# marcelm/cutadapt

Hardware: NVIDIA H100
Metric: reads/sec (150bp SE, 1 adapter, e=0.1) (higher is better)
Workload: dtype u8

## Files before the change

### __graft_entry__.py

```python
import os
import subprocess
import sys

ROOT = os.path.dirname(os.path.abspath(__file__))
CSRC = os.path.join(ROOT, "cutadapt_b200", "csrc")
LIB = os.path.join(ROOT, "cutadapt_b200", "libcutadapt_b200.so")
SOURCES = ["cg_kernels.cu", "cg_fastq.cu", "cg_gzip.cu", "cg_gunzip.cu", "cg_bam.cu", "cg_api.cu", "cg_setbuild.cpp", "cg_host_algos.cpp", "cg_hostpack.cpp", "cg_jit.cpp"]
JIT_HEADERS = ["cg_types.h", "cg_core.cuh", "cg_args.h", "cg_device.cuh", "cg_pscan.cuh"]
HEADERS = ["cg_types.h", "cg_core.cuh", "cg_args.h", "cg_device.cuh", "cg_pscan.cuh", "cg_fastq_core.cuh", "cg_gzip_core.cuh", "cg_gunzip_core.cuh", "cg_bam_core.cuh", "cg_names_core.cuh", "cg_kernels.cuh", "cg_setbuild.h", "cg_hostpack.h", "../../include/cutadapt_b200.h"]


def _newer(target, deps):
    if not os.path.exists(target):
        return True
    t = os.path.getmtime(target)
    return any(os.path.getmtime(d) > t for d in deps if os.path.exists(d))


def write_jit_embed():
    out = os.path.join(CSRC, "cg_jit_embed.h")
    parts = ["// generated by __graft_entry__.write_jit_embed() from " + ", ".join(JIT_HEADERS) + " -- do not edit\n"]
    for i, h in enumerate(JIT_HEADERS):
        text = open(os.path.join(CSRC, h)).read()
        parts.append(f"static const char cg_jit_text_{i}[] =\n")
# ... 33 lines not shown
                print(" ".join(cmd))
            procs.append((cmd, subprocess.Popen(cmd)))
    for cmd, pr in procs:
        if pr.wait() != 0:
            raise subprocess.CalledProcessError(pr.returncode, cmd)
    if force or procs or _newer(LIB, objs):
        subprocess.check_call([nvcc, "-gencode", "arch=compute_90a,code=sm_90a", "-shared", "-o", LIB] + objs
                              + ["-lpthread", "-ldl"])
    return LIB


def build_hostsim(force=False):
    out = os.path.join(ROOT, "tests", "hostsim", "libhostsim.so")
    write_jit_embed()
    srcs = [os.path.join(ROOT, "tests", "hostsim", "hostsim.cpp"), os.path.join(ROOT, "tests", "hostsim", "hostsim_fasta.cpp"),
            os.path.join(ROOT, "tests", "hostsim", "hostsim_route.cpp"),
            os.path.join(ROOT, "tests", "hostsim", "hostsim_pairs.cpp"), os.path.join(ROOT, "tests", "hostsim", "hostsim_gzip.cpp"),
            os.path.join(ROOT, "tests", "hostsim", "hostsim_gunzip.cpp"),
            os.path.join(ROOT, "tests", "hostsim", "hostsim_gunzip_blocks.cpp"),
            os.path.join(ROOT, "tests", "hostsim", "hostsim_quality.cpp"),
            os.path.join(ROOT, "tests", "hostsim", "hostsim_revcomp.cpp"),
            os.path.join(ROOT, "tests", "hostsim", "hostsim_bam.cpp"),
            os.path.join(ROOT, "tests", "hostsim", "hostsim_names.cpp"),
            os.path.join(CSRC, "cg_setbuild.cpp"),
            os.path.join(CSRC, "cg_jit.cpp")]
    deps = srcs + [os.path.join(CSRC, h) for h in ("cg_types.h", "cg_core.cuh", "cg_fastq_core.cuh", "cg_gzip_core.cuh", "cg_gunzip_core.cuh", "cg_bam_core.cuh", "cg_names_core.cuh", "cg_setbuild.h",
                                                   "cg_jit.h", "cg_jit_embed.h")]
    if force or _newer(out, deps):
        subprocess.check_call(["g++", "-O2", "-std=c++17", "-DCG_RUN_BAND=1", "-shared", "-fPIC", "-o", out] + srcs + ["-ldl"])
    return out


def build(force=False):
    build_library(force)
    sys.path.insert(0, ROOT)
    from oracle import oracle as _oracle

    _oracle.build(force)
    build_hostsim(force)
    if os.path.isdir(os.path.join(os.environ.get("CUTADAPT_REFERENCE", ""), "src", "cutadapt")):
        from oracle import build_ref

        build_ref.build()
    import cutadapt_b200
    from cutadapt_b200 import _lib

# ... 42 lines not shown
```

### cutadapt_b200/_lib.py

```python
import ctypes as C
import os
import threading
from typing import Iterable, List, Optional, Sequence, Tuple

import numpy as np

_HERE = os.path.dirname(os.path.abspath(__file__))
LIB_PATH = os.path.join(_HERE, "libcutadapt_b200.so")

CG_OK = 0
CG_EINVAL = -1
CG_ENONASCII = -2
CG_ECUDA = -3
CG_ENOMEM = -4
CG_EUNSUPPORTED = -5
CG_ENOQUAL = -6

CG_KIND_ALIGNER = 0
CG_KIND_PREFIX_COMPARER = 1
CG_KIND_SUFFIX_COMPARER = 2
CG_REMOVE_BEFORE = 0
CG_REMOVE_AFTER = 1
CG_REMOVE_AUTO = 2
CG_GROUP_SINGLE = 0
# ... 201 lines not shown
    lib.cg_fastq_submit_gzip_paired.argtypes = [vp, i32, i32, vp, i64, vp, i64, i32, i32, C.POINTER(i32), C.POINTER(i32),
                                                C.POINTER(cg_gzin_result), C.POINTER(cg_gzin_result)]
    lib.cg_fastq_submit_gzip_interleaved.argtypes = [vp, i32, vp, i64, i32, i32, C.POINTER(i32), C.POINTER(i32),
                                                     C.POINTER(cg_gzin_result)]
    lib.cg_fastq_collect_paired_interleaved.argtypes = [vp, i32, i32, vp, vp, C.POINTER(cg_fastq_params),
                                                        C.POINTER(cg_fastq_params), i32, i32, i32, i32, vp, i64, vp, i64,
                                                        C.POINTER(cg_fastq_result), C.POINTER(cg_fastq_result), vp, vp]
    lib.cg_fastq_stats_create.argtypes = [vp, i32, C.POINTER(i32)]
    lib.cg_fastq_stats_read.argtypes = [vp, i32, C.POINTER(i32), C.POINTER(i32), vp, i64, C.POINTER(i64), C.c_int]
    lib.cg_fastq_stats_destroy.argtypes = [vp, i32]
    lib.cg_names_create.argtypes = [vp, C.POINTER(cg_names_desc), C.POINTER(i32)]
    lib.cg_names_set_mate.argtypes = [vp, i32, i32, C.c_char_p, vp, i32, vp, i32, i32]
    lib.cg_names_destroy.argtypes = [vp, i32]
    lib.cg_adapterset_create.argtypes = [
        vp, C.POINTER(cg_adapter_desc), i32, C.POINTER(cg_group_desc), i32, C.POINTER(vp),
    ]
    lib.cg_adapterset_create_indexed.argtypes = [
        vp, C.POINTER(cg_adapter_desc), i32, C.POINTER(cg_group_desc), i32,
        C.POINTER(cg_index_desc), i32, C.POINTER(vp),
    ]
    lib.cg_adapterset_destroy.argtypes = [vp]
    lib.cg_ctx_stage_times.argtypes = [vp, C.POINTER(C.c_double), C.c_int]
    lib.cg_adapterset_jit_status.argtypes = [vp]
    lib.cg_adapterset_jit_source.argtypes = [vp, C.c_int32, C.c_int32, C.c_int32, C.c_char_p, C.c_int64]
    lib.cg_adapterset_jit_source.restype = C.c_int64
    lib.cg_adapterset_slots.argtypes = [vp]
    lib.cg_adapterset_effective_length.argtypes = [vp, i32, C.POINTER(i32)]
    lib.cg_process_batch.argtypes = [vp, vp, vp, vp, vp, i64, C.POINTER(cg_params), vp, vp]
    lib.cg_process_batch_device.argtypes = [
        vp, vp, vp, vp, vp, i64, i32, C.POINTER(cg_params), vp, vp,
    ]
    lib.cg_process_batch_device_stats.argtypes = [
        vp, vp, vp, vp, vp, i64, i32, C.POINTER(cg_params), vp, vp, i32, i32, vp,
    ]
    lib.cg_kmers_present_batch.argtypes = [vp, C.POINTER(cg_kmer_entry), vp, i32, vp, vp, i64, vp]
    lib.cg_quality_trim_batch.argtypes = [vp, vp, vp, i64, i32, i32, i32, vp]
    lib.cg_nextseq_trim_batch.argtypes = [vp, vp, vp, vp, i64, i32, i32, vp]
    lib.cg_poly_a_trim_batch.argtypes = [vp, vp, vp, i64, i32, vp]
    lib.cg_expected_errors_batch.argtypes = [vp, vp, vp, i64, i32, vp]
    lib.cg_stats_size.argtypes = [i32, i32, i32]
    lib.cg_stats_size.restype = i64
    lib.cg_stats_accumulate_device.argtypes = [
        vp, vp, vp, vp, i64, C.POINTER(cg_params), vp, vp, i32, i32, vp,
    ]
    lib.cg_locate_debug.argtypes = [vp, C.POINTER(cg_adapter_desc), vp, i32, vp, vp, vp]
    lib.cg_process_batch_stats.argtypes = [vp, vp, vp, vp, vp, i64, C.POINTER(cg_params), vp, vp, i32, i32, vp]
    lib.cg_edit_environment.argtypes = [vp, i32, i32, i32, vp, vp, vp, vp, i64]
# ... 315 lines not shown

class AdapterSet:

    def __init__(self, spec: AdapterSetSpec, ctx: Optional[Context] = None):
        self.spec = spec
        self.ctx = ctx or default_context()
        arr, n, garr, ng = spec.to_ctypes()
        handle = C.c_void_p()
        iarr, ni = spec.index_ctypes()
        if ni:
            check(lib().cg_adapterset_create_indexed(self.ctx.handle, arr, n, garr, ng, iarr, ni, C.byref(handle)))
        else:
            check(lib().cg_adapterset_create(self.ctx.handle, arr, n, garr, ng, C.byref(handle)))
        self._h = handle
        self.slots = int(lib().cg_adapterset_slots(handle))

    @property
    def handle(self):
        return self._h

    def jit_status(self) -> int:
        return int(lib().cg_adapterset_jit_status(self._h))

    def jit_source(self, plane_words: int = 5, has_qual: bool = False, statistics: bool = False) -> str:
        n = int(lib().cg_adapterset_jit_source(self._h, plane_words, int(has_qual), int(statistics), None, 0))
        if n == 0:
            return ""
        buf = C.create_string_buffer(n + 1)
        lib().cg_adapterset_jit_source(self._h, plane_words, int(has_qual), int(statistics), buf, n + 1)
        return buf.value.decode()

    def effective_length(self, adapter: int = 0) -> int:
        out = C.c_int32()
        check(lib().cg_adapterset_effective_length(self._h, adapter, C.byref(out)))
        return out.value

    def process(
        self,
        seq: np.ndarray,
        offsets: np.ndarray,
        qual: Optional[np.ndarray] = None,
        params: Optional[cg_params] = None,
        want_qtrim: bool = False,
    ):
        params = params or make_params()
        n = int(offsets.size - 1)
        seq = np.ascontiguousarray(seq, dtype=np.uint8)
        offsets = np.ascontiguousarray(offsets, dtype=np.int64)
        if (params.quality_trim or params.nextseq_trim) and qual is None:
            from .qualtrim import HasNoQualities

            raise HasNoQualities("Cannot do quality trimming when no qualities are available")
# ... 28 lines not shown
```

### cutadapt_b200/csrc/cg_api.cu

```cuda
#include <cuda_runtime.h>
#include <stdio.h>
#include <stdlib.h>
#include <ctype.h>
#include <string.h>

#include <algorithm>
#include <chrono>
#include <map>
#include <memory>
#include <string>
#include <type_traits>
#include <vector>

#include "../../include/cutadapt_b200.h"
#include "cg_hostpack.h"
#include <array>

#include "cg_gzip_core.cuh"
#include "cg_kernels.cuh"
#include "cg_jit.h"
#include "cg_setbuild.h"

static_assert(sizeof(cg_match) == 32 && sizeof(cg_match_rec) == 32, "cg_match must be 32 bytes");
static_assert(sizeof(CgAdapter) == 80 && sizeof(CgEntry) == 32 && sizeof(CgGroup) == 32 &&
// ... 228 lines not shown
    std::map<int32_t, GzinStream> gzin;
    std::map<int32_t, NamesProg> names;
    int32_t names_next = 1;
    int32_t gzin_next = 1;
};

struct cg_adapterset {
    cg_ctx *ctx = nullptr;
    CgBuiltSet host;
    uint8_t *d_blob = nullptr;
    uint64_t *d_masks = nullptr;
    CgEntry *d_entries = nullptr;
    uint8_t *d_index = nullptr;
    struct Pass {
        cg_adapterset *sub = nullptr;
        int group = 0, role = 0;
        int front_pass = -1;
        int map_off = 0;
    };
    std::vector<Pass> passes;
    std::vector<int32_t> pass_map;
    int32_t *d_pass_map = nullptr;
    CgSelectTables select_tables;
    mutable CgJitKernel *jit[2][2][2] = {};
    mutable int jit_state[2][2][2] = {};
    mutable long long plane_reads = 0;
    mutable std::string jit_error;
};

extern "C" int cg_ctx_create(int device, void *stream, cg_ctx **out)
{
    if (!out) return fail(CG_EINVAL, "cg_ctx_create: out is NULL");
    int count = 0;
    cudaError_t e = cudaGetDeviceCount(&count);
    if (e != cudaSuccess || count == 0)
        return fail(CG_ECUDA, std::string("no usable CUDA device (") + cudaGetErrorString(e) +
                                  "); cutadapt_b200 has no CPU fallback");
    if (device < 0 || device >= count) return fail(CG_EINVAL, "cg_ctx_create: device ordinal out of range");
    CU(cudaSetDevice(device));
    std::unique_ptr<cg_ctx, decltype(&cg_ctx_destroy)> c(new cg_ctx(), cg_ctx_destroy);
    c->device = device;
    cudaDeviceProp prop;
    CU(cudaGetDeviceProperties(&prop, device));
    c->sm_count = prop.multiProcessorCount;
    c->smem_optin = prop.sharedMemPerBlockOptin;
    if (stream) { c->stream = (cudaStream_t)stream; c->own_stream = false; }
    else { CU(cudaStreamCreateWithFlags(&c->stream, cudaStreamNonBlocking)); c->own_stream = true; }
    for (int i = 0; i < CG_N_LANES; ++i) CU(cudaStreamCreateWithFlags(&c->lanes[i].stream, cudaStreamNonBlocking));
// ... 155 lines not shown
            if (e == cudaSuccess)
                e = cudaMemcpy(s->d_pass_map, s->pass_map.data(), s->pass_map.size() * sizeof(int32_t), cudaMemcpyHostToDevice);
            if (e != cudaSuccess) { cudaGetLastError(); ok = false; }
        }
        if (!ok) destroy_passes(s);
    }
    *out = s;
    return CG_OK;
}

extern "C" int cg_adapterset_create(cg_ctx *c, const cg_adapter_desc *adapters, int32_t n_adapters,
                                    const cg_group_desc *groups, int32_t n_groups, cg_adapterset **out)
{
    return cg_adapterset_create_indexed(c, adapters, n_adapters, groups, n_groups, nullptr, 0, out);
}

extern "C" int cg_adapterset_destroy(cg_adapterset *s)
{
    if (!s) return CG_OK;
    if (s->ctx) cudaSetDevice(s->ctx->device);
    if (s->d_blob) cudaFree(s->d_blob);
    if (s->d_masks) cudaFree(s->d_masks);
    if (s->d_index) cudaFree(s->d_index);
    for (int w = 0; w < 2; ++w)
        for (int q = 0; q < 2; ++q)
            for (int v = 0; v < 2; ++v) cg_jit_destroy(s->jit[w][q][v]);
    destroy_passes(s);
    delete s;
    return CG_OK;
}

extern "C" int cg_adapterset_jit_status(const cg_adapterset *s)
{
    if (!s) return 0;
    const cg_adapterset *t = (!s->passes.empty() && s->passes[0].sub) ? s->passes[0].sub : s;
    int st = 0;
    for (int w = 0; w < 2; ++w)
        for (int q = 0; q < 2; ++q)
            for (int v = 0; v < 2; ++v) {
                if (t->jit_state[w][q][v] == 1) st = 1;
                else if (t->jit_state[w][q][v] == -1 && st == 0) st = -1;
            }
    if (st == -1) g_err = "first-stage specialisation failed: " + t->jit_error;
    return st;
}

extern "C" int64_t cg_adapterset_jit_source(const cg_adapterset *s, int32_t plane_words, int32_t has_qual, int32_t stats,
                                            char *buf, int64_t cap)
{
    if (!s) return 0;
    const std::string src = cg_jit_pscan_source(s->host, plane_words, has_qual != 0, stats != 0);
    if (buf && cap > 0) {
        const size_t n = std::min<size_t>(src.size(), (size_t)cap - 1);
        memcpy(buf, src.data(), n);
        buf[n] = 0;
    }
    return (int64_t)src.size();
}

extern "C" int cg_adapterset_slots(const cg_adapterset *s) { return s ? s->host.slots : 0; }

extern "C" int cg_adapterset_effective_length(const cg_adapterset *s, int32_t adapter, int32_t *out)
{
    if (!s || !out || adapter < 0 || adapter >= s->host.n_adapters) return fail(CG_EINVAL, "bad adapter index");
    *out = s->host.effective_length[adapter];
    return CG_OK;
}

struct TrimSwitches {
    static bool is(const char *name, const char *value) { const char *e = getenv(name); return e && strcmp(e, value) == 0; }
    static long long at_least_1024(const char *e) { const long long v = e ? atoll(e) : 0; return v >= 1024 ? v : 0; }
    bool force_general = is("CUTADAPT_B200_KERNEL", "general");
    bool force_block = is("CUTADAPT_B200_KERNEL", "block");
    bool force_warp = is("CUTADAPT_B200_KERNEL", "warp");
// ... 75 lines not shown
    d.mini_cap = (int)mini;
    d.carry_slot = (int)(d.plane_w ? std::max<long long>(cslot, 16LL * (2 * d.plane_w + 1) + 16) : cslot);
    size_t scan_smem = d.plane_w ? cg_pscan_smem_bytes(blob_bytes, d.mini_cap, want_q)
                                 : cg_scan_smem_bytes(blob_bytes, d.mini_cap, want_q);
    d.list_smem = cg_dp_smem_bytes(blob_bytes, d.carry_slot);
    if (scan_smem > c->smem_optin || d.list_smem > c->smem_optin) return CG_OK;
    int scan_occ = 0;
    if (d.plane_w) CU(cg_pscan_occupancy(want_q, d.plane_w, false, scan_smem, &scan_occ));
    else CU(cg_scan_occupancy(want_q, scan_smem, &scan_occ));
    CU(cg_list_occupancy(true, h.max_m, false, d.list_smem, &d.plan_occ));
    CU(cg_list_occupancy(false, h.max_m, false, d.list_smem, &d.run_occ));
    if (scan_occ < 1 || d.plan_occ < 1 || d.run_occ < 1) return CG_OK;
    if (d.plane_w && stats && !has_view && h.n_adapters == 1 && times == 1 && h.slots == 1 && !want_q && !sw.two_lists &&
        stats->max_len <= 4096 && cg_stats_entries_smem_bytes(stats->max_len, stats->kmax) <= 48 * 1024) {
        const size_t fsmem = cg_pscan_smem_bytes(blob_bytes, d.mini_cap, want_q, stats->max_len);
        int focc = 0;
        if (fsmem <= c->smem_optin) CU(cg_pscan_occupancy(want_q, d.plane_w, true, fsmem, &focc));
        int pocc = 0, rocc = 0;
        CU(cg_list_occupancy(true, h.max_m, true, d.list_smem, &pocc));
        CU(cg_list_occupancy(false, h.max_m, true, d.list_smem, &rocc));
        d.fuse_stats = focc >= 1 && focc >= scan_occ && pocc >= d.plan_occ && rocc >= d.run_occ;
        if (d.fuse_stats) { scan_smem = fsmem; scan_occ = focc; }
    }
    if (d.plane_w) {
        const int wi = d.plane_w <= 5 ? 0 : 1, qi = want_q ? 1 : 0, vi = d.fuse_stats ? 1 : 0;
        s->plane_reads += n_reads;
        if (!sw.jit_never && s->jit_state[wi][qi][vi] == 0 && (sw.jit_always || s->plane_reads >= (4LL << 20))) {
            std::string err;
            s->jit[wi][qi][vi] = cg_jit_build_pscan(h, d.plane_w, want_q, d.fuse_stats, err);
            s->jit_state[wi][qi][vi] = s->jit[wi][qi][vi] ? 1 : -1;
            if (!s->jit[wi][qi][vi]) s->jit_error = err;
        }
        if (!sw.jit_never && s->jit_state[wi][qi][vi] == 1) {
            d.jit_occ = cg_jit_occupancy(s->jit[wi][qi][vi], CG_NT, scan_smem);
            if (d.jit_occ >= 1) d.jit = s->jit[wi][qi][vi];
        }
    }
    d.kind = TrimKind::Split;
    d.smem = scan_smem; d.occ = scan_occ;
    d.sub = sw.sub_reads ? sw.sub_reads : (d.plane_w && sw.task_bytes) ? (16LL << 20) : (32LL << 20);
    d.sub = std::min<long long>(d.sub, 1LL << 31);
    d.plane_rec = d.plane_w ? (sw.task_bytes ? 4 + 2 * d.plane_w + 1 : 4) : 2;
    return CG_OK;
}

static int trim_grid(const cg_ctx *c, int blocks_per_sm, long long need)
{
    return (int)std::max<long long>(1, std::min<long long>((long long)blocks_per_sm * c->sm_count, need));
}

static int launch_index(cg_ctx *c, const CgKernelArgs &a, const TrimSchedule &d, cudaStream_t st)
{
    int rc = c->tasks.ensure((size_t)((std::min<long long>(a.n_reads, d.sub) + 3) / 4));
    if (rc != CG_OK) return rc;
    for (long long r0 = 0; r0 < a.n_reads; r0 += d.sub) {
        const long long n_sub = std::min<long long>(d.sub, a.n_reads - r0);
        CgKernelArgs b = a;
        b.offsets = a.offsets + r0; b.n_reads = n_sub; b.out = a.out + (size_t)r0 * a.slots;
// ... 3379 lines not shown
```

### cutadapt_b200/csrc/cg_core.cuh

```cuda
#pragma once
#include "cg_types.h"

#define CGK_KIND_ALIGNER 0
#define CGK_KIND_PREFIX 1
#define CGK_KIND_SUFFIX 2
#define CGK_REMOVE_BEFORE 0
#define CGK_REMOVE_AFTER 1
#define CGK_REMOVE_AUTO 2
#define CGK_GROUP_SINGLE 0
#define CGK_GROUP_LINKED 1
#define CGK_GROUP_INDEXED 2

CG_HD int cg_ctz(uint32_t x)
{
#if defined(__CUDA_ARCH__)
    return __ffs((int)x) - 1;
#else
    return __builtin_ctz(x);
#endif
}
CG_HD uint32_t cg_funnel_r(uint32_t lo, uint32_t hi, uint32_t shift_bits)
{
#if defined(__CUDA_ARCH__)
    return __funnelshift_r(lo, hi, shift_bits);
// ... 728 lines not shown
        const int e_min = 32 * W - window + len - 1;
#pragma unroll
        for (int b = 0; b < W; ++b) {
            const int fv = e_min - 32 * b;
            x[b] &= fv <= 0 ? 0xFFFFFFFFu : (fv >= 32 ? 0u : (0xFFFFFFFFu << fv));
        }
#pragma unroll
        for (int b = (W >= 3 ? W - 3 : 0); b < W; ++b) any |= x[b];
    } else {
#pragma unroll
        for (int b = 0; b < W; ++b) any |= x[b];
    }
    if ((flags & (int)CG_PLANE_GUARD) && any) st.guard = true;
    if ((flags & (int)CG_PLANE_PASS) && any) st.pass = true;
    if (flags & (int)CG_PLANE_LOC) {
        if (any) st.anyhit = true;
        if (plane_shl<W>(x, (uint32_t)shift)) st.end_hit = true;
#pragma unroll
        for (int b = 0; b < W; ++b) { st.M[b] |= x[b]; st.E[b] &= x[b]; }
    }
}

struct RuntimePlaneProg {
    CG_HD static bool same_adapter(const uint8_t *w, const uint8_t *ref, int m)
    {
        bool same = true;
        for (int i = 0; i < m; ++i) same = same && ((w[i] & 0xDFu) == ref[i]);
        return same;
    }
    CG_HD static int adapter_length(int m) { return m; }
    CG_HD static unsigned long long overlap_ok(unsigned long long from_blob) { return from_blob; }
    CG_HD static int remove_kind(int from_blob) { return from_blob; }
    template <int W>
    CG_HD static void run(PlaneState<W> &st, const uint32_t *ops, int n_ops, int m)
    {
        const CgPlaneEmit *emits = (const CgPlaneEmit *)((const uint8_t *)ops + (((size_t)n_ops * 4 + 7) & ~(size_t)7));
        for (int i = 0; i < n_ops; ++i) {
            const uint32_t op = ops[i];
            plane_chain_step<W>(st, op & 3u, (op & CG_PLANE_OP_NEW) != 0);
            uint32_t em = op >> 8;
            while (em) {
                const CgPlaneEmit K = emits[(em & 255u) - 1u];
                em >>= 8;
                plane_emit<W>(st, (int)K.len, (int)K.type, (int)K.flags, m - (int)K.bend, (int)K.window);
            }
        }
// ... 1493 lines not shown
```

### cutadapt_b200/csrc/cg_jit.cpp

```cpp
#include "cg_jit.h"

#include <dlfcn.h>
#include <stdio.h>
#include <stdlib.h>
#include <string.h>

#include <mutex>
#include <vector>

#include "cg_jit_embed.h"

typedef struct _nvrtcProgram *nvrtcProgram;
typedef int nvrtcResult;
typedef int CUresult;
typedef struct CUmod_st *CUmodule;
typedef struct CUfunc_st *CUfunction;
typedef struct CUctx_st *CUcontext;
typedef struct CUstream_st *CUstream;

namespace {

struct Api {
    bool tried = false, ok = false;
    std::string why;
// ... 54 lines not shown
    const uint32_t *ops = (const uint32_t *)(set.blob.data() + H->plane_off);
    const int n_ops = H->plane_count;
    const CgPlaneEmit *emits = (const CgPlaneEmit *)((const uint8_t *)ops + (((size_t)n_ops * 4 + 7) & ~(size_t)7));
    std::string t;
    char line[160];
    static const char letters[4] = {'A', 'C', 'T', 'G'};
    for (int i = 0; i < n_ops; ++i) {
        const uint32_t op = ops[i];
        snprintf(line, sizeof line, "        plane_chain_step<W>(st, %uu, %s);   // %c\n", op & 3u,
                 (op & CG_PLANE_OP_NEW) ? "true" : "false", letters[op & 3u]);
        t += line;
        for (uint32_t em = op >> 8; em; em >>= 8) {
            const CgPlaneEmit &K = emits[(em & 255u) - 1u];
            snprintf(line, sizeof line, "        plane_emit<W>(st, %d, %d, %d, %d, %d);\n", (int)K.len, (int)K.type, (int)K.flags,
                     A[0].m - (int)K.bend, (int)K.window);
            t += line;
        }
    }
    return t;
}

}

std::string cg_jit_pscan_source(const CgBuiltSet &set, int W, bool has_qual, bool stats)
{
    const CgSetHeader *H = (const CgSetHeader *)set.blob.data();
    if (H->plane_count <= 0) return std::string();
    std::string src;
    src += "// generated by cg_jit.cpp: the bit-plane first stage specialised for one adapter set\n";
    src += "#include \"cg_pscan.cuh\"\n\n";
    src += "struct StaticPlaneProg {\n";
    src += "    template <int W>\n";
    src += "    __device__ __forceinline__ static void run(PlaneState<W> &st, const uint32_t *, int, int)\n    {\n";
    src += program_text(set);
    src += "    }\n";
    {
        const CgAdapter *A = (const CgAdapter *)(set.blob.data() + H->adapters_off);
        const uint8_t *ref = set.blob.data() + H->pool_off + A[0].ref_off;
        char line[160];
        src += "    // do the first n characters at w spell the adapter's first n (either case)?\n";
        src += "    __device__ __forceinline__ static bool same_adapter(const uint8_t *w, const uint8_t *, int n)\n    {\n";
        src += "        uint32_t diff = 0;\n";
        for (int i = 0; i < A[0].m; ++i) {
            snprintf(line, sizeof line, "        if (%d < n) diff |= (w[%d] & 0xDFu) ^ 0x%02Xu;   // %c\n", i, i, (unsigned)ref[i], (char)ref[i]);
            src += line;
        }
        src += "        return diff == 0;\n    }\n";
        snprintf(line, sizeof line, "    __device__ __forceinline__ static int adapter_length(int) { return %d; }\n", A[0].m);
        src += line;
        src += "    __device__ __forceinline__ static unsigned long long overlap_ok(unsigned long long from_blob) { return from_blob; }\n";
        snprintf(line, sizeof line, "    __device__ __forceinline__ static int remove_kind(int) { return %d; }\n", (int)A[0].remove);
        src += line;
    }
    src += "};\n\n";
    char line[256];
    snprintf(line, sizeof line,
             "extern \"C\" __global__ void __launch_bounds__(CG_NT, %d) cg_pscan_jit(const CgKernelArgs a)\n{\n"
             "    cg_pscan_body<%s, %d, StaticPlaneProg%s>(a);\n}\n",
             W <= 5 ? 8 : 5, has_qual ? "true" : "false", W, stats ? ", true" : "");
    src += line;
    return src;
}

static bool compile(const CgBuiltSet &set, int W, bool has_qual, bool stats, std::vector<char> &cubin, std::string &log)
{
    Api &a = api();
    if (!a.ok) { log = a.why; return false; }
    const std::string src = cg_jit_pscan_source(set, W, has_qual, stats);
    if (src.empty()) { log = "the adapter set has no plane program"; return false; }
    nvrtcProgram prog = nullptr;
    if (a.nvrtcCreateProgram(&prog, src.c_str(), "cg_pscan_jit.cu", cg_jit_n_headers, cg_jit_header_texts, cg_jit_header_names) != 0) {
        log = "nvrtcCreateProgram failed"; return false;
    }
    std::vector<std::string> extra;
    if (const char *defs = getenv("CUTADAPT_B200_JIT_DEFINES")) {
        std::string word;
        for (const char *q = defs;; ++q) {
            if (*q == ' ' || *q == 0) { if (!word.empty()) extra.push_back(word); word.clear(); if (!*q) break; }
            else word.push_back(*q);
        }
    }
    std::vector<const char *> opts = {"--gpu-architecture=sm_90a", "--std=c++17", "-lineinfo"};
    for (const std::string &e : extra) opts.push_back(e.c_str());
    const nvrtcResult rc = a.nvrtcCompileProgram(prog, (int)opts.size(), opts.data());
    size_t n = 0;
    a.nvrtcGetProgramLogSize(prog, &n);
    if (n > 1) { log.resize(n); a.nvrtcGetProgramLog(prog, &log[0]); }
    bool ok = rc == 0;
    if (ok) {
        size_t sz = 0;
        ok = a.nvrtcGetCUBINSize(prog, &sz) == 0 && sz > 0;
        if (ok) { cubin.resize(sz); ok = a.nvrtcGetCUBIN(prog, cubin.data()) == 0; }
        if (!ok) log += " (no cubin)";
        if (ok) {
            if (const char *dump = getenv("CUTADAPT_B200_JIT_DUMP")) {
                if (FILE *f = fopen(dump, "wb")) { fwrite(cubin.data(), 1, cubin.size(), f); fclose(f); }
            }
        }
    }
    a.nvrtcDestroyProgram(&prog);
    return ok;
}

long cg_jit_compile_only(const CgBuiltSet &set, int W, bool has_qual, std::string &log, bool stats)
{
    std::vector<char> cubin;
    if (!compile(set, W, has_qual, stats, cubin, log)) return -1;
    return (long)cubin.size();
}

struct CgJitKernel {
    CUmodule mod = nullptr;
    CUfunction fn = nullptr;
    size_t smem_set = 0;
};

CgJitKernel *cg_jit_build_pscan(const CgBuiltSet &set, int W, bool has_qual, bool stats, std::string &err)
{
    Api &a = api();
    std::vector<char> cubin;
    if (!compile(set, W, has_qual, stats, cubin, err)) return nullptr;
    if (!a.cuda_ok) { err = "libcuda.so.1 not available"; return nullptr; }
    CUcontext cur = nullptr;
    if (a.cuCtxGetCurrent(&cur) != 0 || !cur) { err = "no current CUDA context"; return nullptr; }
    CgJitKernel *k = new CgJitKernel();
    CUresult rc = a.cuModuleLoadData(&k->mod, cubin.data());
    if (rc == 0) rc = a.cuModuleGetFunction(&k->fn, k->mod, "cg_pscan_jit");
    if (rc != 0) {
        char b[64]; snprintf(b, sizeof b, "loading the compiled module failed (CUresult %d)", rc);
        err = b;
        if (k->mod) a.cuModuleUnload(k->mod);
        delete k;
        return nullptr;
    }
    return k;
}

void cg_jit_destroy(CgJitKernel *k)
{
    if (!k) return;
    if (k->mod) api().cuModuleUnload(k->mod);
    delete k;
}

// ... 20 lines not shown
```

### cutadapt_b200/csrc/cg_jit.h

```cpp
#pragma once
#include <stdint.h>
#include <string>

#include "cg_setbuild.h"

struct CgJitKernel;

CgJitKernel *cg_jit_build_pscan(const CgBuiltSet &set, int W, bool has_qual, bool stats, std::string &err);
void cg_jit_destroy(CgJitKernel *k);
std::string cg_jit_pscan_source(const CgBuiltSet &set, int W, bool has_qual, bool stats = false);
int cg_jit_occupancy(CgJitKernel *k, int block, size_t smem);
int cg_jit_launch(CgJitKernel *k, int grid, int block, size_t smem, void *stream, const void *args);
long cg_jit_compile_only(const CgBuiltSet &set, int W, bool has_qual, std::string &log, bool stats = false);
```

### cutadapt_b200/csrc/cg_pscan.cuh

```cuda
#pragma once
#include "cg_core.cuh"
#include "cg_args.h"
#include "cg_device.cuh"

struct ScanSmem { size_t blob_off, enc_off, stats_off, warp_off, warp_stride, bar_rel, seq_rel, qual_rel, total; };

#define CG_PSCAN_MARGIN 272
#ifndef CG_PSCAN_BLOCKS
#define CG_PSCAN_BLOCKS 8
#endif
#define CG_TASK_RESCAN 0x100u
#define CG_TASK_BYTES 0x400u
#define CG_TASK_PLANES 0x200u
struct StatsSmem { uint32_t *hlen, *hrem, *hadj; unsigned long long *scal; };
__host__ __device__ inline size_t stats_smem_bytes(int max_len, int cols)
{
    return cg_align_up((size_t)((1 + 2 * cols) * (max_len + 1) + 8) * sizeof(uint32_t), 8) + 8 * sizeof(unsigned long long);
}
__device__ __forceinline__ StatsSmem stats_smem_view(uint8_t *base, int max_len, int cols)
{
    StatsSmem H;
    H.hlen = (uint32_t *)base;
    H.hrem = H.hlen + (max_len + 1);
    H.hadj = H.hrem + 2 * cols * (max_len + 1);
// ... 116 lines not shown
        if (lane == T) res = resT;
    }
    return res;
#else
    return 0;
#endif
}

__device__ __forceinline__ void pre_trim_warp(const uint8_t *seq, const uint8_t *qual, int n, int flags, int cutoff_front,
                                              int cutoff_back, int qbase, int lane, int *s_out, int *e_out)
{
    const int base = qbase & 255;
    int start = 0, stop = n;
    if (flags & 2) stop = nextseq_trim_core(seq, qual, n, qbase >> 8, base);
    if (flags & 1) {
        const uint32_t q_smem = (uint32_t)__cvta_generic_to_shared(qual);
        const int nq = stop;
        start = trim_scan_warp<+1>(q_smem, nq, cutoff_front, base, lane);
        stop = trim_scan_warp<-1>(q_smem, nq, cutoff_back, base, lane);
        if (start >= stop) { start = 0; stop = 0; }
    }
    *s_out = start; *e_out = stop;
}

template <bool HAS_QUAL, int W, class Prog, bool STATS = false>
__device__ __forceinline__ void cg_pscan_body(const CgKernelArgs &a)
{
    extern __shared__ __align__(128) uint8_t smem[];
    const ScanSmem L = pscan_smem_layout(a.blob_bytes, a.mini_cap, HAS_QUAL, (STATS && a.stats) ? a.stats_max_len : -1);
    uint8_t *s_blob = smem + L.blob_off;
    uint8_t *s_enc = smem + L.enc_off;
    const int tid = threadIdx.x, lane = tid & 31, wib = tid >> 5;
    uint8_t *wbase = smem + L.warp_off + (size_t)wib * L.warp_stride;
    uint64_t *bars = (uint64_t *)(wbase + L.bar_rel);
    uint8_t *s_seq = wbase + L.seq_rel;
    uint8_t *s_qual = wbase + L.qual_rel;
#define CG_PSCAN_STATS_VIEW                                                                                              \
    const int st_len = a.stats_max_len;                                                                                  \
    const StatsSmem H = stats_smem_view(smem + pscan_smem_layout(a.blob_bytes, a.mini_cap, HAS_QUAL, st_len).stats_off, st_len, 1);
    if (STATS && a.stats) {
        CG_PSCAN_STATS_VIEW
        stats_smem_zero(H, st_len, 1);
    }
    for (uint32_t i = tid; i < a.blob_bytes / 16; i += CG_NT) ((uint4 *)s_blob)[i] = ((const uint4 *)a.blob)[i];
    for (uint32_t i = tid; i < 768 / 16; i += CG_NT) ((uint4 *)s_enc)[i] = ((const uint4 *)a.enc)[i];
    if (lane == 0) {
// ... 35 lines not shown
    uint32_t phase0 = 0;
    for (long long mt = wg; mt < n_mt; mt += warps_total) {
        const long long r0 = mt * 32;
        const long long r1 = (r0 + 32 < n_reads) ? r0 + 32 : n_reads;
        const long long r = r0 + lane;
        const long long b0 = a.offsets[r0], b1 = a.offsets[r1];
        long long o0 = 0, o1 = 0;
        if (r < n_reads) { o0 = a.offsets[r]; o1 = a.offsets[r + 1]; }
        const uintptr_t sa0 = (seq_base + b0) & ~(uintptr_t)15;
        if (b1 > b0) { mbar_wait(&bars[0], phase0); phase0 ^= 1; }
        int q_ts = 0, q_te = 0;
        if (HAS_QUAL && a.quality_trim) {
            const uintptr_t qa0 = (qual_base + b0) & ~(uintptr_t)15;
            const bool has = r < n_reads;
            pre_trim_warp(s_seq + (size_t)(has ? (seq_base + o0) - sa0 : 0), s_qual + (size_t)(has ? (qual_base + o0) - qa0 : 0),
                          has ? (int)(o1 - o0) : 0, a.quality_trim, a.cutoff_front, a.cutoff_back, a.qbase, lane, &q_ts, &q_te);
        }
        int cls = CG_PLANE_NONE, s0 = 0, ts = 0, te = 0;
        int st_fin = -1;
        uint32_t st_p1 = 0, st_p2 = 0, st_p3 = 0;
        uint32_t t_flags = 4u | CG_TASK_RESCAN;
        uint32_t tm[8] = {0, 0, 0, 0, 0, 0, 0, 0};
        uint32_t win_region = 0, win_off = 0;
        bool mine = false;
        if (r < n_reads) {
            mine = true;
            const int n = (int)(o1 - o0);
            const uint32_t off = (uint32_t)((seq_base + o0) - sa0);
            ts = 0; te = n;
            if (HAS_QUAL && a.quality_trim) { ts = q_ts; te = q_te; }
            if (a.qtrim) { a.qtrim[2 * r] = ts; a.qtrim[2 * r + 1] = te; }
            if (a.view) { ts = a.view[2 * r]; te = a.view[2 * r + 1]; }
            const int nn = te - ts;
            if (nn >= 1 && nn <= 32 * W) {
                const PlaneOut po = plane_scan_core<W, Prog>(prog, n_prog, pflags, A.m, ref, s_seq + off + te, nn, always_pass);
                cls = po.cls; s0 = po.s0;
                if (po.bad & 0x80808080u) atomicOr(a.err_flag, 1);
                if (cls == CG_PLANE_SLOW) {
                    t_flags = 4u | CG_TASK_PLANES | (a.task_rec > 4 ? CG_TASK_BYTES : 0u) | ((uint32_t)W << 12) |
                              ((uint32_t)po.end_hit << 20) | ((uint32_t)po.no_end << 21);
                    const uint32_t wend = smem_u32(s_seq + off + te);
                    win_region = (wend - 32u * W) & ~15u;
                    win_off = (wend - (uint32_t)nn) - win_region;
#pragma unroll
                    for (int b = 0; b < 8; ++b) tm[b] = po.M[b];
                }
            } else {
                cls = CG_PLANE_SLOW;
                uint32_t bad = 0;
                for (int i = ts; i < te; ++i) bad |= s_seq[off + i];
                if (bad & 0x80u) atomicOr(a.err_flag, 1);
            }
            if (cls != CG_PLANE_SLOW) {
                CgHit hit; hit.adapter = -1; hit.remove = 0;
                hit.astart = hit.astop = hit.rstart = hit.rstop = hit.score = hit.errors = 0;
                if (cls == CG_PLANE_EXACT) hit_exact(A, nn, s0, hit);
                else if (cls == CG_PLANE_OVERLAP) hit_end_overlap(A, nn, s0, hit);
                store_hit(a.out + (size_t)r * a.slots, hit, 0, nn);
// ... 4 lines not shown
                    int fin = nn;
                    if (hit.adapter >= 0) {
                        const int kind = Prog::remove_kind(A.remove);
                        const bool after = kind == CGK_REMOVE_AUTO ? hit.remove == CGK_REMOVE_AFTER : kind == CGK_REMOVE_AFTER;
                        int removed = after ? nn - hit.rstart : hit.rstop;
                        removed = removed < 0 ? 0 : removed;
                        st_p2 |= (uint32_t)removed | (1u << 22);
                        atomicAdd(&H.hrem[(after ? st_len + 1 : 0) + (removed > st_len ? st_len : removed)], 1u);
                        if (after) {
                            int k = 4;
                            if (hit.rstart > 0) {
                                const uint8_t c = s_seq[off + ts + hit.rstart - 1];
                                k = c == 'A' ? 0 : (c == 'C' ? 1 : (c == 'G' ? 2 : (c == 'T' ? 3 : 4)));
                            }
                            st_p3 = 1u << (6 * k);
                            fin = hit.rstart;
                        } else {
                            fin = nn - hit.rstop;
                        }
                    }
                    st_fin = fin < 0 ? 0 : (fin > st_len ? st_len : fin);
                }
            }
        }
        if (STATS && a.stats) {
            CG_PSCAN_STATS_VIEW
            stats_warp_add(H, st_fin, st_p1, st_p2, st_p3);
        }
        const bool slow = mine && cls == CG_PLANE_SLOW;
        const bool kind_b = slow && a.task_count_b != nullptr && (t_flags & CG_TASK_PLANES) && !(t_flags & (1u << 20)) &&
                            (tm[0] | tm[1] | tm[2] | tm[3] | tm[4] | tm[5] | tm[6] | tm[7]) == 0u;
        const uint32_t ballot_a = __ballot_sync(0xffffffffu, slow && !kind_b);
        const uint32_t ballot_b = __ballot_sync(0xffffffffu, kind_b);
        if (ballot_a | ballot_b) {
            unsigned long long base_a = 0, base_b = 0;
            if (lane == 0) {
                if (ballot_a) base_a = atomicAdd(a.task_count, (unsigned long long)__popc(ballot_a));
                if (ballot_b) base_b = atomicAdd(a.task_count_b, (unsigned long long)__popc(ballot_b));
            }
            base_a = __shfl_sync(0xffffffffu, base_a, 0);
            base_b = __shfl_sync(0xffffffffu, base_b, 0);
            if (slow) {
                const uint32_t below = (1u << lane) - 1u;
                const unsigned long long slot = kind_b
                    ? (unsigned long long)a.task_cap - 1ull - (base_b + __popc(ballot_b & below))
                    : base_a + __popc(ballot_a & below);
// ... 31 lines not shown
```

### include/cutadapt_b200.h

```cpp
#ifndef CUTADAPT_B200_H
#define CUTADAPT_B200_H

#include <stddef.h>
#include <stdint.h>

#ifdef __cplusplus
extern "C" {
#endif

#define CG_ABI_VERSION 1

#define CG_OK 0
#define CG_EINVAL (-1)
#define CG_ENONASCII (-2)
#define CG_ECUDA (-3)
#define CG_ENOMEM (-4)
#define CG_EUNSUPPORTED (-5)
#define CG_ENOQUAL (-6)

#define CG_START_IN_REFERENCE 1
#define CG_START_IN_QUERY 2
#define CG_STOP_IN_REFERENCE 4
#define CG_STOP_IN_QUERY 8

// ... 89 lines not shown
int cg_ctx_stage_times(cg_ctx *ctx, double *out3, int reset);

int cg_ctx_transfer_bytes(cg_ctx *ctx, int64_t *h2d, int64_t *d2h, int reset);

int cg_host_cpus_available(void);
int cg_host_threads(void);
int cg_ctx_numa_node(cg_ctx *ctx);

int cg_ctx_host_profile(cg_ctx *ctx, double *out, int reset);

int cg_adapterset_create(cg_ctx *ctx, const cg_adapter_desc *adapters, int32_t n_adapters,
                         const cg_group_desc *groups, int32_t n_groups, cg_adapterset **out);
int cg_adapterset_create_indexed(cg_ctx *ctx, const cg_adapter_desc *adapters, int32_t n_adapters,
                                 const cg_group_desc *groups, int32_t n_groups,
                                 const cg_index_desc *indexes, int32_t n_indexes, cg_adapterset **out);
#define CG_DEBUG_NONE (-2147483647 - 1)
int cg_locate_debug(cg_ctx *ctx, const cg_adapter_desc *adapter, const uint8_t *query, int32_t n,
                    int32_t *cost, int32_t *score, int32_t *result8);

int cg_adapterset_destroy(cg_adapterset *set);

int cg_adapterset_jit_status(const cg_adapterset *set);
int64_t cg_adapterset_jit_source(const cg_adapterset *set, int32_t plane_words, int32_t has_qual, int32_t stats,
                                 char *buf, int64_t cap);
int cg_adapterset_slots(const cg_adapterset *set);
int cg_adapterset_effective_length(const cg_adapterset *set, int32_t adapter, int32_t *out);

int cg_process_batch(cg_ctx *ctx, const cg_adapterset *set, const uint8_t *seq,
                     const uint8_t *qual, const int64_t *offsets, int64_t n_reads,
                     const cg_params *params, cg_match *matches, int32_t *qtrim);
int cg_process_batch_device(cg_ctx *ctx, const cg_adapterset *set, const uint8_t *d_seq,
                            const uint8_t *d_qual, const int64_t *d_offsets, int64_t n_reads,
                            int32_t max_read_len, const cg_params *params, cg_match *d_matches,
                            int32_t *d_qtrim);
int cg_process_batch_device_stats(cg_ctx *ctx, const cg_adapterset *set, const uint8_t *d_seq, const uint8_t *d_qual,
                                  const int64_t *d_offsets, int64_t n_reads, int32_t max_read_len, const cg_params *params,
                                  cg_match *d_matches, int32_t *d_qtrim, int32_t stats_max_len, int32_t stats_kmax,
                                  int64_t *d_stats);

int64_t cg_pack3_host(const uint8_t *seq, int64_t a0, int64_t lo, int64_t hi, int64_t n_stream,
                      uint8_t *packed, uint64_t *exceptions, int64_t capacity, int32_t n_threads);

int cg_kmers_present_batch(cg_ctx *ctx, const cg_kmer_entry *entries, const uint64_t *masks,
                           int32_t n_entries, const uint8_t *seq, const int64_t *offsets,
                           int64_t n_reads, uint8_t *out);
int cg_quality_trim_batch(cg_ctx *ctx, const uint8_t *qual, const int64_t *offsets,
                          int64_t n_reads, int32_t cutoff_front, int32_t cutoff_back,
// ... 202 lines not shown
```

Before: 7.565 billion.

## Specialise JIT plane-scan kernel on a compile-time read length

The NVRTC-compiled first-stage kernel now also takes the batch's max read length as a constexpr. When a whole warp holds reads of exactly that length, it takes a path with constant length and offsets, so the compiler can fold loop bounds and addressing. The JIT cache becomes a vector keyed by (width, qual, stats, length), with at most four length variants per configuration. It also adds -default-device to the NVRTC options. The cost is more JIT compiles, plus a second inlined copy of the per-read body that can raise register pressure.

Result: no change. 7.633 billion (median of 6 runs) (+0.9%).

```diff
diff --git a/__graft_entry__.py b/__graft_entry__.py
--- a/__graft_entry__.py
+++ b/__graft_entry__.py
@@ -79,6 +79,7 @@
             os.path.join(ROOT, "tests", "hostsim", "hostsim_revcomp.cpp"),
             os.path.join(ROOT, "tests", "hostsim", "hostsim_bam.cpp"),
             os.path.join(ROOT, "tests", "hostsim", "hostsim_names.cpp"),
+            os.path.join(ROOT, "tests", "hostsim", "hostsim_jit.cpp"),
             os.path.join(CSRC, "cg_setbuild.cpp"),
             os.path.join(CSRC, "cg_jit.cpp")]
     deps = srcs + [os.path.join(CSRC, h) for h in ("cg_types.h", "cg_core.cuh", "cg_fastq_core.cuh", "cg_gzip_core.cuh", "cg_gunzip_core.cuh", "cg_bam_core.cuh", "cg_names_core.cuh", "cg_setbuild.h",
diff --git a/cutadapt_b200/_lib.py b/cutadapt_b200/_lib.py
--- a/cutadapt_b200/_lib.py
+++ b/cutadapt_b200/_lib.py
@@ -247,7 +247,7 @@
     lib.cg_adapterset_destroy.argtypes = [vp]
     lib.cg_ctx_stage_times.argtypes = [vp, C.POINTER(C.c_double), C.c_int]
     lib.cg_adapterset_jit_status.argtypes = [vp]
-    lib.cg_adapterset_jit_source.argtypes = [vp, C.c_int32, C.c_int32, C.c_int32, C.c_char_p, C.c_int64]
+    lib.cg_adapterset_jit_source.argtypes = [vp, C.c_int32, C.c_int32, C.c_int32, C.c_int32, C.c_char_p, C.c_int64]
     lib.cg_adapterset_jit_source.restype = C.c_int64
     lib.cg_adapterset_slots.argtypes = [vp]
     lib.cg_adapterset_effective_length.argtypes = [vp, i32, C.POINTER(i32)]
@@ -609,12 +609,12 @@
     def jit_status(self) -> int:
         return int(lib().cg_adapterset_jit_status(self._h))
 
-    def jit_source(self, plane_words: int = 5, has_qual: bool = False, statistics: bool = False) -> str:
-        n = int(lib().cg_adapterset_jit_source(self._h, plane_words, int(has_qual), int(statistics), None, 0))
+    def jit_source(self, plane_words: int = 5, has_qual: bool = False, statistics: bool = False, read_len: int = 0) -> str:
+        n = int(lib().cg_adapterset_jit_source(self._h, plane_words, int(has_qual), int(statistics), read_len, None, 0))
         if n == 0:
             return ""
         buf = C.create_string_buffer(n + 1)
-        lib().cg_adapterset_jit_source(self._h, plane_words, int(has_qual), int(statistics), buf, n + 1)
+        lib().cg_adapterset_jit_source(self._h, plane_words, int(has_qual), int(statistics), read_len, buf, n + 1)
         return buf.value.decode()
 
     def effective_length(self, adapter: int = 0) -> int:
diff --git a/cutadapt_b200/csrc/cg_api.cu b/cutadapt_b200/csrc/cg_api.cu
--- a/cutadapt_b200/csrc/cg_api.cu
+++ b/cutadapt_b200/csrc/cg_api.cu
@@ -274,8 +274,8 @@
     std::vector<int32_t> pass_map;
     int32_t *d_pass_map = nullptr;
     CgSelectTables select_tables;
-    mutable CgJitKernel *jit[2][2][2] = {};
-    mutable int jit_state[2][2][2] = {};
+    struct Jit { int w, q, v, len; CgJitKernel *k; int state; };
+    mutable std::vector<Jit> jit;
     mutable long long plane_reads = 0;
     mutable std::string jit_error;
 };
@@ -477,9 +477,7 @@
     if (s->d_blob) cudaFree(s->d_blob);
     if (s->d_masks) cudaFree(s->d_masks);
     if (s->d_index) cudaFree(s->d_index);
-    for (int w = 0; w < 2; ++w)
-        for (int q = 0; q < 2; ++q)
-            for (int v = 0; v < 2; ++v) cg_jit_destroy(s->jit[w][q][v]);
+    for (const cg_adapterset::Jit &j : s->jit) cg_jit_destroy(j.k);
     destroy_passes(s);
     delete s;
     return CG_OK;
@@ -490,21 +488,19 @@
     if (!s) return 0;
     const cg_adapterset *t = (!s->passes.empty() && s->passes[0].sub) ? s->passes[0].sub : s;
     int st = 0;
-    for (int w = 0; w < 2; ++w)
-        for (int q = 0; q < 2; ++q)
-            for (int v = 0; v < 2; ++v) {
-                if (t->jit_state[w][q][v] == 1) st = 1;
-                else if (t->jit_state[w][q][v] == -1 && st == 0) st = -1;
-            }
+    for (const cg_adapterset::Jit &j : t->jit) {
+        if (j.state == 1) st = 1;
+        else if (j.state == -1 && st == 0) st = -1;
+    }
     if (st == -1) g_err = "first-stage specialisation failed: " + t->jit_error;
     return st;
 }
 
 extern "C" int64_t cg_adapterset_jit_source(const cg_adapterset *s, int32_t plane_words, int32_t has_qual, int32_t stats,
-                                            char *buf, int64_t cap)
+                                            int32_t read_len, char *buf, int64_t cap)
 {
     if (!s) return 0;
-    const std::string src = cg_jit_pscan_source(s->host, plane_words, has_qual != 0, stats != 0);
+    const std::string src = cg_jit_pscan_source(s->host, plane_words, has_qual != 0, stats != 0, read_len);
     if (buf && cap > 0) {
         const size_t n = std::min<size_t>(src.size(), (size_t)cap - 1);
         memcpy(buf, src.data(), n);
@@ -626,18 +622,31 @@
         d.fuse_stats = focc >= 1 && focc >= scan_occ && pocc >= d.plan_occ && rocc >= d.run_occ;
         if (d.fuse_stats) { scan_smem = fsmem; scan_occ = focc; }
     }
-    if (d.plane_w) {
-        const int wi = d.plane_w <= 5 ? 0 : 1, qi = want_q ? 1 : 0, vi = d.fuse_stats ? 1 : 0;
-        s->plane_reads += n_reads;
-        if (!sw.jit_never && s->jit_state[wi][qi][vi] == 0 && (sw.jit_always || s->plane_reads >= (4LL << 20))) {
+    if (d.plane_w) s->plane_reads += n_reads;
+    if (d.plane_w && !sw.jit_never) {
+        const int q = want_q ? 1 : 0, v = d.fuse_stats ? 1 : 0;
+        auto find = [&](int len) -> cg_adapterset::Jit * {
+            for (cg_adapterset::Jit &j : s->jit)
+                if (j.w == d.plane_w && j.q == q && j.v == v && j.len == len) return &j;
+            return nullptr;
+        };
+        int len = want_q ? 0 : max_read_len;
+        cg_adapterset::Jit *j = find(len);
+        if (!j && len > 0) {
+            int lengths = 0;
+            for (const cg_adapterset::Jit &e : s->jit) lengths += e.w == d.plane_w && e.q == q && e.v == v && e.len > 0;
+            if (lengths >= 4) { len = 0; j = find(0); }
+        }
+        if (!j && (sw.jit_always || s->plane_reads >= (4LL << 20))) {
             std::string err;
-            s->jit[wi][qi][vi] = cg_jit_build_pscan(h, d.plane_w, want_q, d.fuse_stats, err);
-            s->jit_state[wi][qi][vi] = s->jit[wi][qi][vi] ? 1 : -1;
-            if (!s->jit[wi][qi][vi]) s->jit_error = err;
+            CgJitKernel *k = cg_jit_build_pscan(h, d.plane_w, want_q, d.fuse_stats, len, err);
+            if (!k) s->jit_error = err;
+            s->jit.push_back({d.plane_w, q, v, len, k, k ? 1 : -1});
+            j = &s->jit.back();
         }
-        if (!sw.jit_never && s->jit_state[wi][qi][vi] == 1) {
-            d.jit_occ = cg_jit_occupancy(s->jit[wi][qi][vi], CG_NT, scan_smem);
-            if (d.jit_occ >= 1) d.jit = s->jit[wi][qi][vi];
+        if (j && j->state == 1) {
+            d.jit_occ = cg_jit_occupancy(j->k, CG_NT, scan_smem);
+            if (d.jit_occ >= 1) d.jit = j->k;
         }
     }
     d.kind = TrimKind::Split;
diff --git a/cutadapt_b200/csrc/cg_core.cuh b/cutadapt_b200/csrc/cg_core.cuh
--- a/cutadapt_b200/csrc/cg_core.cuh
+++ b/cutadapt_b200/csrc/cg_core.cuh
@@ -774,6 +774,7 @@
 }
 
 struct RuntimePlaneProg {
+    static constexpr int read_len = 0;
     CG_HD static bool same_adapter(const uint8_t *w, const uint8_t *ref, int m)
     {
         bool same = true;
diff --git a/cutadapt_b200/csrc/cg_jit.cpp b/cutadapt_b200/csrc/cg_jit.cpp
--- a/cutadapt_b200/csrc/cg_jit.cpp
+++ b/cutadapt_b200/csrc/cg_jit.cpp
@@ -100,7 +100,7 @@
 
 }
 
-std::string cg_jit_pscan_source(const CgBuiltSet &set, int W, bool has_qual, bool stats)
+std::string cg_jit_pscan_source(const CgBuiltSet &set, int W, bool has_qual, bool stats, int read_len)
 {
     const CgSetHeader *H = (const CgSetHeader *)set.blob.data();
     if (H->plane_count <= 0) return std::string();
@@ -108,6 +108,11 @@
     src += "// generated by cg_jit.cpp: the bit-plane first stage specialised for one adapter set\n";
     src += "#include \"cg_pscan.cuh\"\n\n";
     src += "struct StaticPlaneProg {\n";
+    {
+        char line[96];
+        snprintf(line, sizeof line, "    static constexpr int read_len = %d;\n", read_len);
+        src += line;
+    }
     src += "    template <int W>\n";
     src += "    __device__ __forceinline__ static void run(PlaneState<W> &st, const uint32_t *, int, int)\n    {\n";
     src += program_text(set);
@@ -140,11 +145,12 @@
     return src;
 }
 
-static bool compile(const CgBuiltSet &set, int W, bool has_qual, bool stats, std::vector<char> &cubin, std::string &log)
+static bool compile(const CgBuiltSet &set, int W, bool has_qual, bool stats, int read_len, std::vector<char> &cubin,
+                    std::string &log)
 {
     Api &a = api();
     if (!a.ok) { log = a.why; return false; }
-    const std::string src = cg_jit_pscan_source(set, W, has_qual, stats);
+    const std::string src = cg_jit_pscan_source(set, W, has_qual, stats, read_len);
     if (src.empty()) { log = "the adapter set has no plane program"; return false; }
     nvrtcProgram prog = nullptr;
     if (a.nvrtcCreateProgram(&prog, src.c_str(), "cg_pscan_jit.cu", cg_jit_n_headers, cg_jit_header_texts, cg_jit_header_names) != 0) {
@@ -158,7 +164,7 @@
             else word.push_back(*q);
         }
     }
-    std::vector<const char *> opts = {"--gpu-architecture=sm_90a", "--std=c++17", "-lineinfo"};
+    std::vector<const char *> opts = {"--gpu-architecture=sm_90a", "--std=c++17", "-lineinfo", "-default-device"};
     for (const std::string &e : extra) opts.push_back(e.c_str());
     const nvrtcResult rc = a.nvrtcCompileProgram(prog, (int)opts.size(), opts.data());
     size_t n = 0;
@@ -180,10 +186,10 @@
     return ok;
 }
 
-long cg_jit_compile_only(const CgBuiltSet &set, int W, bool has_qual, std::string &log, bool stats)
+long cg_jit_compile_only(const CgBuiltSet &set, int W, bool has_qual, std::string &log, bool stats, int read_len)
 {
     std::vector<char> cubin;
-    if (!compile(set, W, has_qual, stats, cubin, log)) return -1;
+    if (!compile(set, W, has_qual, stats, read_len, cubin, log)) return -1;
     return (long)cubin.size();
 }
 
@@ -193,11 +199,11 @@
     size_t smem_set = 0;
 };
 
-CgJitKernel *cg_jit_build_pscan(const CgBuiltSet &set, int W, bool has_qual, bool stats, std::string &err)
+CgJitKernel *cg_jit_build_pscan(const CgBuiltSet &set, int W, bool has_qual, bool stats, int read_len, std::string &err)
 {
     Api &a = api();
     std::vector<char> cubin;
-    if (!compile(set, W, has_qual, stats, cubin, err)) return nullptr;
+    if (!compile(set, W, has_qual, stats, read_len, cubin, err)) return nullptr;
     if (!a.cuda_ok) { err = "libcuda.so.1 not available"; return nullptr; }
     CUcontext cur = nullptr;
     if (a.cuCtxGetCurrent(&cur) != 0 || !cur) { err = "no current CUDA context"; return nullptr; }
diff --git a/cutadapt_b200/csrc/cg_jit.h b/cutadapt_b200/csrc/cg_jit.h
--- a/cutadapt_b200/csrc/cg_jit.h
+++ b/cutadapt_b200/csrc/cg_jit.h
@@ -6,9 +6,9 @@
 
 struct CgJitKernel;
 
-CgJitKernel *cg_jit_build_pscan(const CgBuiltSet &set, int W, bool has_qual, bool stats, std::string &err);
+CgJitKernel *cg_jit_build_pscan(const CgBuiltSet &set, int W, bool has_qual, bool stats, int read_len, std::string &err);
 void cg_jit_destroy(CgJitKernel *k);
-std::string cg_jit_pscan_source(const CgBuiltSet &set, int W, bool has_qual, bool stats = false);
+std::string cg_jit_pscan_source(const CgBuiltSet &set, int W, bool has_qual, bool stats = false, int read_len = 0);
 int cg_jit_occupancy(CgJitKernel *k, int block, size_t smem);
 int cg_jit_launch(CgJitKernel *k, int grid, int block, size_t smem, void *stream, const void *args);
-long cg_jit_compile_only(const CgBuiltSet &set, int W, bool has_qual, std::string &log, bool stats = false);
+long cg_jit_compile_only(const CgBuiltSet &set, int W, bool has_qual, std::string &log, bool stats = false, int read_len = 0);
diff --git a/cutadapt_b200/csrc/cg_pscan.cuh b/cutadapt_b200/csrc/cg_pscan.cuh
--- a/cutadapt_b200/csrc/cg_pscan.cuh
+++ b/cutadapt_b200/csrc/cg_pscan.cuh
@@ -162,6 +162,8 @@
     }
     *s_out = start; *e_out = stop;
 }
+
+template <int N> struct CgIntConst { static constexpr int value = N; };
 
 template <bool HAS_QUAL, int W, class Prog, bool STATS = false>
 __device__ __forceinline__ void cg_pscan_body(const CgKernelArgs &a)
@@ -243,18 +245,20 @@
         uint32_t t_flags = 4u | CG_TASK_RESCAN;
         uint32_t tm[8] = {0, 0, 0, 0, 0, 0, 0, 0};
         uint32_t win_region = 0, win_off = 0;
-        bool mine = false;
-        if (r < n_reads) {
-            mine = true;
-            const int n = (int)(o1 - o0);
-            const uint32_t off = (uint32_t)((seq_base + o0) - sa0);
+        bool uniform = false;
+        if (!HAS_QUAL && Prog::read_len > 0)
+            uniform = __all_sync(0xffffffffu, r < n_reads && o1 - o0 == Prog::read_len) && a.view == nullptr;
+        auto settle = [&](auto len_tag) {
+            constexpr int NC = decltype(len_tag)::value;
+            const int n = NC ? NC : (int)(o1 - o0);
+            const uint32_t off = NC ? ((uint32_t)(seq_base + b0) & 15u) + (uint32_t)lane * NC : (uint32_t)((seq_base + o0) - sa0);
             ts = 0; te = n;
             if (HAS_QUAL && a.quality_trim) { ts = q_ts; te = q_te; }
             if (a.qtrim) { a.qtrim[2 * r] = ts; a.qtrim[2 * r + 1] = te; }
-            if (a.view) { ts = a.view[2 * r]; te = a.view[2 * r + 1]; }
-            const int nn = te - ts;
+            if (!NC && a.view) { ts = a.view[2 * r]; te = a.view[2 * r + 1]; }
+            const int nn = NC ? NC : te - ts;
             if (nn >= 1 && nn <= 32 * W) {
-                const PlaneOut po = plane_scan_core<W, Prog>(prog, n_prog, pflags, A.m, ref, s_seq + off + te, nn, always_pass);
+                const PlaneOut po = plane_scan_core<W, Prog>(prog, n_prog, pflags, A.m, ref, s_seq + off + (NC ? NC : te), nn, always_pass);
                 cls = po.cls; s0 = po.s0;
                 if (po.bad & 0x80808080u) atomicOr(a.err_flag, 1);
                 if (cls == CG_PLANE_SLOW) {
@@ -305,6 +309,12 @@
                     st_fin = fin < 0 ? 0 : (fin > st_len ? st_len : fin);
                 }
             }
+        };
+        bool mine = false;
+        if (r < n_reads) {
+            mine = true;
+            if (uniform) settle(CgIntConst<Prog::read_len>{});
+            else settle(CgIntConst<0>{});
         }
         if (STATS && a.stats) {
             CG_PSCAN_STATS_VIEW
diff --git a/include/cutadapt_b200.h b/include/cutadapt_b200.h
--- a/include/cutadapt_b200.h
+++ b/include/cutadapt_b200.h
@@ -135,7 +135,7 @@
 
 int cg_adapterset_jit_status(const cg_adapterset *set);
 int64_t cg_adapterset_jit_source(const cg_adapterset *set, int32_t plane_words, int32_t has_qual, int32_t stats,
-                                 char *buf, int64_t cap);
+                                 int32_t read_len, char *buf, int64_t cap);
 int cg_adapterset_slots(const cg_adapterset *set);
 int cg_adapterset_effective_length(const cg_adapterset *set, int32_t adapter, int32_t *out);
 
```
